# yifita/iso-points

Hardware: AMD Instinct MI355X
Metric: Mpoints/s full iso-point cycle (project+resample+splat), 1M pts (higher is better)
Workload: dtype f32-class (split-fp16 operands, 2^-22: hidden-layer products from two fp16 parts per f32 operand under exact power-of-two scales, 3 fp16-MFMA passes, f32 accumulate; everything else f32)

## Files before the change

include/isopoints.h:

```cpp
#ifndef ISOPOINTS_H_
#define ISOPOINTS_H_

#include <stdint.h>

#ifdef __cplusplus
extern "C" {
#endif

#define ISO_OK 0
#define ISO_ERR_INVALID (-1)
#define ISO_ERR_UNSUPPORTED (-2)
#define ISO_ERR_LAUNCH (-3)
#define ISO_ERR_WORKSPACE (-4)

const char* iso_version(void);
const char* iso_last_error(void);


int iso_project_sphere(const float* pts_in, float* pts_out, float* normals_out,
                       uint8_t* mask_out, int64_t n, float cx, float cy,
                       float cz, float radius, int max_iters, float tol,
                       void* stream);

typedef struct iso_follow {
// ... 297 lines not shown
int iso_bricks_box_take(void* workspace, int64_t n_max, float* box_out, void* stream);
int iso_bricks_build(const float* points, const float* normals, const int32_t* payload,
                     int64_t n_own, int64_t id_base, const float* import_rec0,
                     const float* import_rec1, const int32_t* import_count, int64_t import_max,
                     const float* bbox, int64_t n_total, float radius, int knn_k,
                     float cell_scale, void* workspace, int64_t workspace_bytes, void* stream);
int iso_bricks_params(const float* boxes, int n_boxes, int64_t n_total, int64_t n_own, int64_t id_base, float radius,
                      int knn_k, float cell_scale, void* workspace, int64_t n_max, void* stream);
int iso_halo_export(void* workspace, const float* points, const float* normals, const int32_t* payload,
                    int64_t n_own, const float* rank_boxes, int world, int rank, int halo_cells,
                    float* export_buf, int64_t capacity, void* stream);
int iso_halo_import(void* workspace, int64_t n_max, const float* gathered, const float* rank_boxes, int world,
                    int rank, int halo_cells, int64_t capacity, float* import_rec0, float* import_rec1,
                    int32_t* import_count, int64_t import_capacity, void* stream);
int iso_resample_fused(void* workspace, int64_t n_max, const float* points, int64_t n_own,
                       int k_plus_one, float* points_out, int64_t* idx_out, float* d2_out,
                       void* stream);
int iso_splat_view_mask(const float* points, const float* normals, const float* views, int n_views,
                        int64_t n, float znear, float zfar, int backface_culling,
                        int32_t* mask_out, int32_t* view_count_out, void* stream);
int iso_splat_h_fused(void* workspace, int64_t n_max, const float* points, const int32_t* mask,
                      int64_t n_own, const int32_t* view_total, int n_views, float* h_out,
                      void* stream);
int64_t iso_splat_front_workspace_bytes(int64_t n_points);
int iso_splat_front(const float* points, const float* normals, const float* features, int channels,
                    int features_from_normals, const int32_t* mask, const float* h, int64_t n_points,
                    const float* views, const float* projs, int n_views, int image_size, float sigma,
                    float cutoff, void* workspace, int64_t workspace_bytes, int64_t* first_idx_out,
                    int64_t* num_pts_out, int32_t* view_total_out, float* ndc_out, float* ellipse_out,
                    float* cutoff_out, float* radii_out, float* scaler_out, float* features_out,
                    int32_t* src_out, void* stream);
int iso_splat_view_mask_scan(const float* points, const float* normals, const float* views, int n_views,
                             int64_t n_points, float znear, float zfar, int backface_culling, int32_t* mask_out,
                             void* workspace, int64_t workspace_bytes, int64_t* first_idx_out, int64_t* num_pts_out,
                             int32_t* view_total_out, void* stream);
int iso_splat_front_rows(const float* points, const float* normals, const float* features, int channels,
                         int features_from_normals, const int32_t* mask, const float* h, int64_t n_points,
                         const float* views, const float* projs, int n_views, int image_size, float sigma,
                         float cutoff, const void* workspace, int64_t workspace_bytes, const int64_t* first_idx,
                         float* ndc_out, float* ellipse_out, float* cutoff_out, float* radii_out,
                         float* scaler_out, float* features_out, int32_t* src_out,
                         uint8_t* visible_zero_out ,
                         int64_t row_capacity ,
                         int32_t* overflow_out ,
                         void* stream);
int iso_splat_points_backward(const float* points, int64_t n_points, const float* views, const float* projs,
// ... 129 lines not shown
```

iso_points_amd/_lib.py:

```python
import ctypes
import os

import torch

_HERE = os.path.dirname(os.path.abspath(__file__))
LIB_PATH = os.path.join(_HERE, "libisopoints_hip.so")
if os.environ.get("ISO_DEV_LIB"):
    LIB_PATH = os.path.abspath(os.environ["ISO_DEV_LIB"])

_c = ctypes
_P = _c.c_void_p
_I = _c.c_int
_L = _c.c_int64
_F = _c.c_float

SIGNATURES = {
    "iso_version": (_c.c_char_p, []),
    "iso_last_error": (_c.c_char_p, []),
    "iso_project_sphere": (_I, [_P, _P, _P, _P, _L, _F, _F, _F, _F, _I, _F, _P]),
    "iso_project_sphere_follow": (_I, [_P, _P, _P, _P, _L, _F, _F, _F, _F, _I, _F, _P, _P]),
    "iso_siren_raw_floats": (_L, [_I, _I]),
    "iso_siren_packed_floats": (_L, [_I, _I]),
    "iso_siren_set_gemm_mode": (_I, [_I]),
    "iso_siren_get_gemm_mode": (_I, []),
# ... 66 lines not shown
                                      _L, _P, _P, _I, _I, _F, _P, _P, _P]),
    "iso_gather_neg_idx": (_I, [_P, _P, _L, _P, _P]),
    "iso_splat_composite": (_I, [_P, _P, _P, _P, _P, _L, _I, _I, _I, _F, _P, _P, _P]),
    "iso_splat_composite_backward": (_I, [_P, _P, _P, _P, _P, _L, _I, _I, _I, _F, _P, _P, _P, _P, _P]),
    "iso_splat_mark_visible": (_I, [_P, _L, _I, _P, _P]),
    "iso_splat_median_radius_workspace_bytes": (_L, [_I]),
    "iso_splat_median_radius": (_I, [_P, _P, _P, _P, _I, _L, _F, _P, _L, _P, _P]),
    "iso_splat_backward_workspace_bytes": (_L, [_I, _I, _I, _L]),
    "iso_splat_backward": (_I, [_P, _P, _P, _P, _P, _P, _I, _L, _P, _P, _P, _I, _I, _I, _I, _F, _L, _P, _L, _P, _P]),
    "iso_splat_zbuf_backward": (_I, [_P, _P, _L, _I, _P, _P]),
    "iso_bricks_workspace_bytes": (_L, [_L]),
    "iso_bricks_workspace_init": (_I, [_P, _L, _P]),
    "iso_bricks_workspace_check": (_I, [_P, _L, _P]),
    "iso_bricks_build_whole": (_I, [_P, _P, _P, _L, _F, _I, _F, _P, _L, _P]),
    "iso_bricks_build_pending": (_I, [_P, _P, _P, _L, _F, _I, _F, _P, _L, _P, _P]),
    "iso_bricks_box_take": (_I, [_P, _L, _P, _P]),
    "iso_bricks_build": (_I, [_P, _P, _P, _L, _L, _P, _P, _P, _L, _P, _L, _F, _I, _F, _P, _L, _P]),
    "iso_bricks_params": (_I, [_P, _I, _L, _L, _L, _F, _I, _F, _P, _L, _P]),
    "iso_halo_export": (_I, [_P, _P, _P, _P, _L, _P, _I, _I, _I, _P, _L, _P]),
    "iso_halo_import": (_I, [_P, _L, _P, _P, _I, _I, _I, _L, _P, _P, _P, _L, _P]),
    "iso_resample_fused": (_I, [_P, _L, _P, _L, _I, _P, _P, _P, _P]),
    "iso_splat_view_mask": (_I, [_P, _P, _P, _I, _L, _F, _F, _I, _P, _P, _P]),
    "iso_splat_h_fused": (_I, [_P, _L, _P, _P, _L, _P, _I, _P, _P]),
    "iso_splat_z_absmax": (_I, [_P, _L, _P, _P]),
    "iso_splat_z_scatter": (_I, [_P, _P, _L, _I, _L, _P, _P, _P]),
    "iso_splat_z_finish": (_I, [_P, _P, _L, _L, _P, _P]),
    "iso_splat_band_marks": (_I, [_P, _P, _I, _L, _L, _I, _P, _P, _P]),
    "iso_splat_band_z_scatter": (_I, [_P, _P, _I, _L, _L, _I, _P, _P, _P]),
    "iso_splat_repack": (_I, [_P, _L, _I, _I, _I, _P, _F, _L, _P, _P, _P, _P, _P, _P, _P, _P, _P, _P, _P]),
    "iso_splat_band_segment_floats": (_L, [_L]),
    "iso_splat_band_export_workspace_bytes": (_L, [_L, _I, _I]),
    "iso_splat_band_export": (_I, [_P, _P, _P, _P, _P, _P, _P, _I, _L, _P, _I, _I, _I, _I, _L, _P, _P, _P, _P, _P, _P, _P, _P,
                                   _P, _L, _P]),
    "iso_splat_band_import": (_I, [_P, _I, _I, _L, _L, _F, _P, _P, _P, _P, _P, _P, _P, _P, _P, _P, _P, _P, _P, _P, _P]),
    "iso_splat_band_remap": (_I, [_P, _P, _I, _L, _L, _L, _I, _P, _P]),
    "iso_splat_band_return": (_I, [_P, _P, _P, _P, _P, _I, _L, _P, _P]),
    "iso_splat_band_merge": (_I, [_P, _P, _I, _I, _L, _L, _P, _P, _P, _P]),
    "iso_splat_median_pass_words": (_L, [_I]),
    "iso_splat_median_pass": (_I, [_I, _P, _P, _P, _P, _I, _L, _P, _L, _P]),
    "iso_splat_median_final": (_I, [_P, _I, _F, _P, _P]),
    "iso_insert_fathers": (_I, [_P, _P, _I, _L, _P, _P, _P, _P, _P]),
    "iso_insert_children": (_I, [_P, _P, _I, _L, _I, _I, _P, _P, _P, _P, _P]),
    "iso_splat_points_backward": (_I, [_P, _L, _P, _P, _I, _P, _P, _P, _P, _P, _P, _P]),
    "iso_rasterize_coarse": (_I, [_P, _P, _P, _P, _I, _I, _I, _I, _P, _P, _P]),
    "iso_rasterize_fine": (_I, [_P, _P, _P, _P, _L, _P, _I, _I, _F, _I, _I, _I, _P, _P, _P, _P, _P]),
    "iso_splat_front_workspace_bytes": (_L, [_L]),
# ... 86 lines not shown
```

iso_points_amd/bricks.py:

```python
import torch

from . import _lib

RESAMPLE_CELL = 0.8
H_CELL_SCALE = 6.0


def points_bbox(points, out=None):
    pts = points.detach().float().contiguous().view(-1, 3)
    mm = out if out is not None else torch.empty((8,), dtype=torch.float32, device=pts.device)
    _lib.call("iso_points_bbox", _lib.ptr(pts), None, 1, pts.shape[0], _lib.ptr(mm), _lib.stream())
    return mm


class BrickGrid(object):

    def __init__(self, n_own, device, import_max=0):
        self.n_own, self.import_max = int(n_own), int(import_max)
        self.n_max = self.n_own + self.import_max
        lib = _lib.load()
        self.ws_bytes = lib.iso_bricks_workspace_bytes(self.n_max)
        self.ws = torch.empty((self.ws_bytes,), dtype=torch.uint8, device=device)
        assert self.ws.data_ptr() % 256 == 0
        _lib.call("iso_bricks_workspace_init", _lib.ptr(self.ws), self.n_max, _lib.stream())
# ... 36 lines not shown
                  p(self.ws), self.ws_bytes, _lib.stream())
        self.points = points
        self._imports = imports
        return self

    def counters_since_last(self):
        c = self.ws[256:384].cpu().view(torch.int32).tolist()
        tot = [(c[i] + c[16 + i]) & 0xffffffff for i in range(16)]
        out = [(tot[i] - self._seen[i]) & 0xffffffff for i in range(16)]
        self._seen = tot
        return out

    def check_initialised(self):
        _lib.call("iso_bricks_workspace_check", _lib.ptr(self.ws), self.n_max, _lib.stream())

    def header(self):
        self.check_initialised()
        raw = self.ws[:128].cpu()
        f = raw.view(torch.float32).tolist()
        i = raw.view(torch.int32).tolist()
        c = self.ws[256:320].cpu().view(torch.int32).tolist()
        return {"f": f[8], "r": f[9], "inv_sigma": f[12], "diag": f[13], "nb": i[16:19], "n_bricks": i[19],
                "n": i[23], "n_own": i[24], "id_base": i[25], "g_covers_r": i[26], "occupied": c[0],
                "tail": c[1], "overflow_bricks": c[2], "tail_h": c[3]}


class Follow(object):

    def __init__(self, grid, n, views=None, znear=1.0, zfar=100.0, backface_culling=True):
        dev = grid.ws.device
        self.grid, self.n = grid, int(n)
        self.done = False
        self.views = None
        self.mask = self.total = self.scanned = None
        self.znear, self.zfar, self.backface = float(znear), float(zfar), bool(backface_culling)
        if views is not None:
            nv = views.shape[0]
            self.views = views.detach().float().contiguous()
            self.mask = torch.empty((self.n,), dtype=torch.int32, device=dev)
            ws = torch.empty((_lib.load().iso_splat_front_workspace_bytes(self.n),), dtype=torch.uint8, device=dev)
            first = torch.empty((nv,), dtype=torch.int64, device=dev)
            num = torch.empty((nv,), dtype=torch.int64, device=dev)
            self.total = torch.empty((8,), dtype=torch.int32, device=dev)
            self.scanned = (ws, first, num, self.total)

    def struct(self):
        p = lambda t: (t.data_ptr() if t is not None else None)
# ... 64 lines not shown
```

iso_points_amd/csrc/bricks.hip:

```cpp
#include <type_traits>
#include "bricks.h"

#pragma clang fp contract(off)

constexpr int kScan1MaxWords = 2048;
BrickWs bricks_carve(void* ws, int64_t n_max) {
  BrickWs w;
  if (n_max < 1) n_max = 1;
  w.nb_cap = bricks_nb_cap(n_max);
  w.G = BK_CPB * (int64_t)w.nb_cap * w.nb_cap * w.nb_cap + 1;
  auto al = [](int64_t b) { return (b + 255) / 256 * 256; };
  char* p = (char*)ws;
  int64_t o = 0;
  w.hdr = (BrickHdr*)(p + o); o += al(sizeof(BrickHdr));
  w.counters = (int32_t*)(p + o); o += al(4 * kCounterInts);
  w.scan1 = (unsigned*)(p + o); o += al(4 * kScan1MaxWords);
  w.cnt = (int32_t*)(p + o); o += al(4 * w.G);
  w.off = (int32_t*)(p + o); o += al(4 * w.G);
  w.slot = (int32_t*)(p + o); o += al(4 * n_max);
  w.rec0 = (float4*)(p + o); o += al(16 * n_max);
  w.rec1 = (float4*)(p + o); o += al(16 * n_max);
  w.list = (int32_t*)(p + o); o += al(4 * (w.G < n_max ? w.G : n_max));
  w.tail = (int32_t*)(p + o); o += al(4 * 8 * n_max);
  w.scan_ws_bytes = iso_prefix_sum_workspace_bytes(w.G, 1) + 4 * (kScan1MaxWords + (w.G + 1023) / 1024);
// ... 666 lines not shown
  constexpr int NL = BrickStage<WITH_NRM, 2>::NL;
  int cell = (wx * NL + wy) * NL + wz;
  int i = S.cstart[cell], e = S.cstart[cell + NW];
  cell += NL;
  int ni = S.cstart[cell], ne = S.cstart[cell + NW];
  int run = 0, m = 1;
  while (run < NW * NW) {
    const bool v0 = i < e, v1 = i + 1 < e;
    const int i0 = v0 ? i : 0, i1 = v1 ? i + 1 : i0;
    const float4 c0 = S.rec0[i0];
    const float4 c1 = S.rec0[i1];
    body(c0, i0, c1, i1, v0, v1);
    i += 2;
    if (i >= e) {
      ++run;
      i = ni; e = ne;
      m = m == NW - 1 ? 0 : m + 1;
      cell += m == 0 ? NL * NL - (NW - 1) * NL : NL;
      if (run < NW * NW - 1) { ni = S.cstart[cell]; ne = S.cstart[cell + NW]; }
    }
  }
}

__device__ void brick_to_tail(const BrickHdr& h, const int32_t* __restrict__ off, const float4* __restrict__ rec0, int b,
                              int32_t* __restrict__ tail, int32_t* __restrict__ counters, int tail_slot, int per_query) {
  for (int i = off[BK_CPB * b] + threadIdx.x; i < off[BK_CPB * (b + 1)]; i += BK_THREADS) {
    const int gid = __float_as_int(rec0[i].w);
    if (gid >= h.id_base && gid < h.id_base + h.n_own) {
      const int at = atomicAdd(&counters[tail_slot], per_query);
      for (int v = 0; v < per_query; ++v) tail[at + v] = per_query > 1 ? (gid - h.id_base) * 8 + v : gid - h.id_base;
    }
  }
  if (threadIdx.x == 0) atomicAdd(&counters[2], 1);
}

struct Repulse {
  float px, py, pz, inv_sigma;
  float sw = 0.f, mx = 0.f, my = 0.f, mz = 0.f;
  __device__ __forceinline__ void add(float qx, float qy, float qz, float ux, float uy, float uz) {
    const float dx = px - qx, dy = py - qy, dz = pz - qz;
    const float d2 = (dx * dx + dy * dy) + dz * dz;
    const float w = expf(-d2 * inv_sigma);
    const float dn = (dx * ux + dy * uy) + dz * uz;
    const float tx = dx - dn * ux, ty = dy - dn * uy, tz = dz - dn * uz;
    sw += w;
    mx += w * tx; my += w * ty; mz += w * tz;
  }
  __device__ __forceinline__ void finish(float* __restrict__ o) const {
    const float dens = sw + 1.0f;
    const float den = iso_eps_denom(sw, 1.0e-17f);
    o[0] = px + dens * mx / den;
    o[1] = py + dens * my / den;
    o[2] = pz + dens * mz / den;
  }
};

__device__ __forceinline__ bool pair_lt(float d1, int i1, float d2, int i2) {
  return d1 < d2 || (d1 == d2 && i1 < i2);
}

constexpr int kXcdChunks = 8;
__device__ __forceinline__ int bk_xcd_span(int n_list) {
  return kXcdChunks * ((n_list + kXcdChunks - 1) / kXcdChunks);
}
__device__ __forceinline__ int bk_xcd_item(int lj, int n_list) {
  const int chunk = (n_list + kXcdChunks - 1) / kXcdChunks;
  return (lj % kXcdChunks) * chunk + lj / kXcdChunks;
}

template <int M>
__global__ __launch_bounds__(BK_THREADS, 4) void k_brick_resample(
    const BrickHdr* __restrict__ hp, const int32_t* __restrict__ off, const int32_t* __restrict__ list,
    const float4* __restrict__ rec0, const float4* __restrict__ rec1, int K, float* __restrict__ out,
    int64_t* __restrict__ idx_out, float* __restrict__ d2_out, int32_t* __restrict__ tail,
    int32_t* __restrict__ counters) {
  __shared__ BrickStage<true, 2> S;
  __shared__ int s_unc[BK_THREADS], s_nunc;
  const BrickHdr h = *hp;
  const int n_list = counters[0];
  for (int lj = blockIdx.x; lj < bk_xcd_span(n_list); lj += gridDim.x) {
    const int li = bk_xcd_item(lj, n_list);
    if (li >= n_list) continue;
    const int b = list[li];
    BrickGeo g;
    if (threadIdx.x == 0) s_nunc = 0;
    const int C = stage_brick<true, 1, 2>(S, h, off, rec0, rec1, b, g);
    if (C < 0) { brick_to_tail(h, off, rec0, b, tail, counters, 1, 1); continue; }
    const int nq = S.qpre[BrickStage<true, 2>::NQRUN];
    auto one_query = [&](int pos, auto wide_tag) -> bool {
      constexpr bool WIDE = decltype(wide_tag)::value;
      constexpr int ML = (WIDE && M == 10) ? 12 : M;
      const float4 q = S.rec0[pos];
      const int gid = __float_as_int(q.w);
      int wx, wy, wz;
      float mfrac = 0.f;
      {
        auto win = [&](float pc, float mn, int nf, int o) {
          const float t2 = ((pc - mn) * h.inv_f) * 2.0f;
          int sc = (int)floorf(t2);
          sc = sc < 0 ? 0 : (sc >= 2 * nf ? 2 * nf - 1 : sc);
          if (WIDE) return 2 * (sc >> 1) - 2 * o - 2;
          const float fr = t2 - (float)sc;
          const bool low = fr < 0.5f;
          mfrac = fmaxf(mfrac, low ? fr : 1.0f - fr);
          return sc - 2 * o - (low ? 2 : 1);
        };
        wx = win(q.x, h.mn[0], h.nf[0], g.ox);
        wy = win(q.y, h.mn[1], h.nf[1], g.oy);
        wz = win(q.z, h.mn[2], h.nf[2], g.oz);
      }
      float gq2 = h.g2;
      if (!WIDE) { const float gq = (2.0f - mfrac) * 0.5f; gq2 = (gq * gq) * h.g2; }
      unsigned key[ML];
#pragma unroll
      for (int j = 0; j < ML; ++j) key[j] = 0xffffffffu;
      auto visit = [&](const float4& c0, int i0, const float4& c1, int i1, bool v0, bool v1) {
        const float da = bk_d2(q.x, q.y, q.z, c0.x, c0.y, c0.z);
        const float db = bk_d2(q.x, q.y, q.z, c1.x, c1.y, c1.z);
        const unsigned ka = v0 ? ((__float_as_uint(da) & ~1023u) | (unsigned)i0) : 0xffffffffu;
        const unsigned kb = v1 ? ((__float_as_uint(db) & ~1023u) | (unsigned)i1) : 0xffffffffu;
#pragma unroll
        for (int j = ML - 1; j >= 1; --j) key[j] = bk_med3u(key[j - 1], ka, key[j]);
        key[0] = min(key[0], ka);
#pragma unroll
        for (int j = ML - 1; j >= 1; --j) key[j] = bk_med3u(key[j - 1], kb, key[j]);
        key[0] = min(key[0], kb);
      };
      if (WIDE) walk_window<6>(S, wx, wy, wz, visit);
      else walk_window_flat<4>(S, wx, wy, wz, visit);
      float d[ML];
      int id[ML], ps[ML];
#pragma unroll
      for (int j = 0; j < ML; ++j) {
        const bool valid = key[j] != 0xffffffffu;
        ps[j] = valid ? (int)(key[j] & 1023u) : pos;
        const float4 c = S.rec0[ps[j]];
        const float d2 = bk_d2(q.x, q.y, q.z, c.x, c.y, c.z);
        const bool ok = valid && d2 < h.r2;
        d[j] = ok ? d2 : FLT_MAX;
        id[j] = ok ? __float_as_int(c.w) : 0x7fffffff;
      }
      bool swapped;
      do {
        swapped = false;
#pragma unroll
        for (int j = 0; j + 1 < ML; ++j) {
          if (pair_lt(d[j + 1], id[j + 1], d[j], id[j])) {
            const float td = d[j]; d[j] = d[j + 1]; d[j + 1] = td;
            const int ti = id[j]; id[j] = id[j + 1]; id[j + 1] = ti;
            const int tp = ps[j]; ps[j] = ps[j + 1]; ps[j + 1] = tp;
            swapped = true;
// ... 20 lines not shown
          if (j < ML && j < K && d[j < ML ? j : 0] < FLT_MAX) u[k] = rec1[S.src[ps[j < ML ? j : 0]]];
        }
#pragma unroll
        for (int k = 0; k < 4; ++k) {
          const int j = j0 + k;
          if (j < ML && j < K && d[j < ML ? j : 0] < FLT_MAX) {
            const float4 c = S.rec0[ps[j < ML ? j : 0]];
            R.add(c.x, c.y, c.z, u[k].x, u[k].y, u[k].z);
          }
        }
      }
      R.finish(out + (int64_t)row * 3);
      if (idx_out) {
#pragma unroll
        for (int j = 1; j < ML; ++j)
          if (j < K) {
            idx_out[(int64_t)row * (K - 1) + j - 1] = d[j] < FLT_MAX ? (int64_t)id[j] : (int64_t)-1;
            if (d2_out) d2_out[(int64_t)row * (K - 1) + j - 1] = d[j] < FLT_MAX ? d[j] : -1.0f;
          }
      }
      return true;
    };
    auto to_tail = [&](int pos) { tail[atomicAdd(&counters[1], 1)] = __float_as_int(S.rec0[pos].w) - h.id_base; };
    for (int t = threadIdx.x; t < nq; t += BK_THREADS) {
      const int pos = query_slot(S, t);
      const int gid = __float_as_int(S.rec0[pos].w);
      if (gid < h.id_base || gid >= h.id_base + h.n_own) continue;
      if (!one_query(pos, std::false_type())) {
        const int at = atomicAdd(&s_nunc, 1);
        if (at < BK_THREADS) s_unc[at] = pos; else to_tail(pos);
      }
    }
    __syncthreads();
    const int n_unc = min(s_nunc, BK_THREADS);
    for (int u = threadIdx.x; u < n_unc; u += BK_THREADS) {
      const int pos = s_unc[u];
      if (!one_query(pos, std::true_type())) to_tail(pos);
    }
  }
}

struct WalkGeo { float qx, qy, qz, mnx, mny, mnz, B; };
constexpr int kWalkItems = 8;

template <class Fetch, class Body, class Bound, class Local>
__device__ __forceinline__ void bk_walk_shell(int rin, int rho, int qbx, int qby, int qbz, int nbx, int nby, int nbz,
                                              const int32_t* __restrict__ off, int lane, const WalkGeo& G,
                                              Fetch&& fetch, Body&& body, Bound&& bound, Local&& local,
                                              int part = 0, int nparts = 1) {
  const int x0 = max(qbx - rho, 0), x1 = min(qbx + rho, nbx - 1);
  const int y0 = max(qby - rho, 0), y1 = min(qby + rho, nby - 1);
  if (x0 > x1 || y0 > y1) return;
  const int ny = y1 - y0 + 1, ncols = (x1 - x0 + 1) * ny;
  for (int c0 = 0; c0 < ncols; c0 += 64) {
    int s0 = 0, e0 = 0, s1 = 0, e1 = 0;
    float dm0 = FLT_MAX, dm1 = FLT_MAX;
    const int col = c0 + lane;
    const float far2 = bound();
    auto gap = [&](float q, float mn, int b0, int b1) {
      const float lo = mn + (float)b0 * G.B, hi = mn + (float)(b1 + 1) * G.B;
// ... 215 lines not shown
  for (int v = 0; v < 8; ++v) {
    if (v < n_views) {
      int c = local[v];
#pragma unroll
      for (int o = 32; o > 0; o >>= 1) c += __shfl_xor(c, o);
      if ((threadIdx.x & 63) == 0 && c) atomicAdd(&s_cnt[v], c);
    }
  }
  __syncthreads();
  if (threadIdx.x < n_views && s_cnt[threadIdx.x]) atomicAdd(&view_count[threadIdx.x], s_cnt[threadIdx.x]);
}

__device__ __forceinline__ float h_from_list(const float* d , bool small_cloud) {
  float m = -FLT_MAX;
#pragma unroll
  for (int k = 1; k < 7; ++k) {
    const float v = small_cloud ? 1e-3f : (d[k] < FLT_MAX ? d[k] : -1.0f);
    m = fmaxf(m, v);
  }
  return fminf(fmaxf(0.5f * m, 5e-5f), 0.01f);
}

constexpr int kHWgs = 6;
template <int NV>
__global__ __launch_bounds__(BK_THREADS, NV <= 4 ? kHWgs : 4) void k_brick_h(
    const BrickHdr* __restrict__ hp, const int32_t* __restrict__ off, const int32_t* __restrict__ list,
    const float4* __restrict__ rec0, const float4* __restrict__ rec1, const int32_t* __restrict__ view_total,
    int n_views, float* __restrict__ h_out , int32_t* __restrict__ tail,
    int32_t* __restrict__ counters) {
  __shared__ BrickStage<false, 1, BK_CAP> S;
  const BrickHdr h = *hp;
  const int n_list = counters[0];
  bool small_cloud[NV];
#pragma unroll
  for (int v = 0; v < NV; ++v) small_cloud[v] = v < n_views && view_total[v] < 7;
  const float kT = 2.0f * 5e-5f;
  const float t2 = fminf(kT, h.r2 > 0.f ? __uint_as_float(__float_as_uint(h.r2) - 1u) : 0.f);
  for (int lj = blockIdx.x; lj < bk_xcd_span(n_list); lj += gridDim.x) {
    const int li = bk_xcd_item(lj, n_list);
    if (li >= n_list) continue;
    const int b = list[li];
    BrickGeo g;
    constexpr int VS = NV <= 4 ? 8 : 1;
    const int C = stage_brick<false, VS, 1, BK_CAP>(S, h, off, rec0, rec1, b, g);
    if (C < 0) { brick_to_tail(h, off, rec0, b, tail, counters, 3, 8); continue; }
    const int nq = S.qpre[16];
    for (int t0 = 0; t0 < nq; t0 += BK_THREADS) {
      const int t = t0 + threadIdx.x;
      float4 q = make_float4(0.f, 0.f, 0.f, 0.f);
      int qmask = 0, lx = 1, ly = 1, lz = 1, row = 0, sx = 1, sy = 1;
      if (t < nq) {
        const int pos = query_slot(S, t);
        q = S.rec0[pos];
        qmask = __float_as_int(q.w);
        if (qmask < 0) qmask = 0;
        row = S.gid[pos] - h.id_base;
        const int fx = bk_fine(q.x, h.mn[0], h.inv_f, h.nf[0]), fy = bk_fine(q.y, h.mn[1], h.inv_f, h.nf[1]);
        lx = fx - g.ox;
        ly = fy - g.oy;
        lz = bk_fine(q.z, h.mn[2], h.inv_f, h.nf[2]) - g.oz;
        sx = ((q.x - h.mn[0]) * h.inv_f - (float)fx) >= 0.5f ? 1 : -1;
        sy = ((q.y - h.mn[1]) * h.inv_f - (float)fy) >= 0.5f ? 1 : -1;
      }
      int cnt[NV];
#pragma unroll
      for (int v = 0; v < NV; ++v) cnt[v] = 0;
      if (VS == 8 && C <= 255) {
        unsigned acc = 0;
        const unsigned need = ((unsigned)qmask & 0x01010101u) << 7;
        if (qmask)
          walk_candidates_near_first(S, lx, ly, lz, sx, sy, [&](const float4& c0, const float4& c1, bool v0, bool v1) {
            const float da = bk_d2(q.x, q.y, q.z, c0.x, c0.y, c0.z);
            const float db = bk_d2(q.x, q.y, q.z, c1.x, c1.y, c1.z);
            const unsigned ma = (v0 && da <= t2) ? (__float_as_uint(c0.w) & 0x01010101u) : 0u;
            const unsigned mb = (v1 && db <= t2) ? (__float_as_uint(c1.w) & 0x01010101u) : 0u;
            acc += ma + mb;
          }, [&]() {
            const unsigned ge7 = (((acc & 0x7f7f7f7fu) + 0x79797979u) | acc) & 0x80808080u;
            return (ge7 & need) == need;
          });
#pragma unroll
        for (int v = 0; v < NV; ++v) cnt[v] = (int)((acc >> (8 * (v & 3))) & 0xffu);
      } else if (qmask)
        walk_candidates_near_first(S, lx, ly, lz, sx, sy, [&](const float4& c0, const float4& c1, bool v0, bool v1) {
          const float da = bk_d2(q.x, q.y, q.z, c0.x, c0.y, c0.z);
          const float db = bk_d2(q.x, q.y, q.z, c1.x, c1.y, c1.z);
          const int ma = (v0 && da <= t2) ? __float_as_int(c0.w) : 0;
          const int mb = (v1 && db <= t2) ? __float_as_int(c1.w) : 0;
#pragma unroll
          for (int v = 0; v < NV; ++v) cnt[v] += ((ma >> (VS * v)) & 1) + ((mb >> (VS * v)) & 1);
        }, [&]() {
          bool all = true;
#pragma unroll
          for (int v = 0; v < NV; ++v) all = all && (!((qmask >> (VS * v)) & 1) || cnt[v] >= 7);
          return all;
        });
      bool open_ = false;
#pragma unroll
      for (int v = 0; v < NV; ++v) open_ = open_ || (((qmask >> (VS * v)) & 1) && !small_cloud[v] && cnt[v] < 7);
      float d[NV][7];
#pragma unroll
      for (int v = 0; v < NV; ++v)
#pragma unroll
        for (int j = 0; j < 7; ++j) d[v][j] = FLT_MAX;
      if (open_)
        walk_candidates(S, lx, ly, lz, [&](const float4& c0, const float4& c1, bool v0, bool v1) {
          float da = bk_d2(q.x, q.y, q.z, c0.x, c0.y, c0.z);
          float db = bk_d2(q.x, q.y, q.z, c1.x, c1.y, c1.z);
          da = (v0 && da < h.r2) ? da : FLT_MAX;
          db = (v1 && db < h.r2) ? db : FLT_MAX;
          const int ma = __float_as_int(c0.w), mb = __float_as_int(c1.w);
#pragma unroll
          for (int v = 0; v < NV; ++v) {
            const float ka = (ma >> (VS * v)) & 1 ? da : FLT_MAX;
            const float kb = (mb >> (VS * v)) & 1 ? db : FLT_MAX;
#pragma unroll
            for (int j = 6; j >= 1; --j) d[v][j] = __builtin_amdgcn_fmed3f(d[v][j - 1], ka, d[v][j]);
            d[v][0] = fminf(d[v][0], ka);
#pragma unroll
            for (int j = 6; j >= 1; --j) d[v][j] = __builtin_amdgcn_fmed3f(d[v][j - 1], kb, d[v][j]);
            d[v][0] = fminf(d[v][0], kb);
          }
        });
      if (qmask) {
#pragma unroll
        for (int v = 0; v < NV; ++v) {
          if (v < n_views && ((qmask >> (VS * v)) & 1)) {
            float hv;
            bool cert = true;
            if (small_cloud[v]) hv = fminf(fmaxf(0.5f * 1e-3f, 5e-5f), 0.01f);
            else if (cnt[v] >= 7) hv = 5e-5f;
            else {
              cert = h.g_covers_r || (d[v][6] < FLT_MAX && d[v][6] <= h.g2);
              hv = h_from_list(d[v], false);
            }
            if (cert) h_out[(int64_t)v * h.n_own + row] = hv;
            else tail[atomicAdd(&counters[3], 1)] = row * 8 + v;
          }
        }
      }
    }
  }
}

template <int KMAX>
struct TopF {
  float d[KMAX];
// ... 417 lines not shown
  ISO_REQUIRE(workspace && gathered && rank_boxes && import_rec0 && import_rec1 && import_count && world >= 1 &&
                  rank >= 0 && rank < world && capacity >= 0 && import_capacity >= 0 && halo_cells >= 1,
              ISO_ERR_INVALID, "iso_halo_import: bad arguments");
  const BrickWs w = bricks_carve(workspace, n_max);
  hipStream_t s = (hipStream_t)stream;
  iso_zero_words(import_count, 1, s);
  if (capacity > 0 && world > 1)
    hipLaunchKernelGGL(k_halo_import, dim3(iso_stream_grid(capacity, 256) > 64 ? 64 : iso_stream_grid(capacity, 256), world),
                       dim3(256), 0, s, (const float4*)gathered, world, rank, (int)capacity, halo_cells, w.hdr, rank_boxes,
                       (float4*)import_rec0, (float4*)import_rec1, import_count, (int)import_capacity, w.counters);
  ISO_CHECK_LAUNCH("iso_halo_import");
  return ISO_OK;
}

static int brick_grid(int64_t n_own, int cap) {
  int64_t g = n_own / 48;
  if (g < 1024) g = 1024;
  if (g > cap) g = cap;
  return (int)g;
}
static int h_grid(int64_t n_own) { return brick_grid(n_own, 10240); }
static int resample_grid(int64_t n_own) { return brick_grid(n_own, 8192); }

extern "C" int iso_resample_fused(void* workspace, int64_t n_max, const float* points, int64_t n_own,
                                  int k_plus_one, float* points_out, int64_t* idx_out, float* d2_out,
                                  void* stream) {
  ISO_REQUIRE(workspace && n_own >= 0 && n_max >= n_own, ISO_ERR_INVALID, "iso_resample_fused: bad arguments");
  ISO_REQUIRE(k_plus_one >= 2 && k_plus_one <= 13, ISO_ERR_UNSUPPORTED,
              "iso_resample_fused: K + 1 must be in [2,13], got %d", k_plus_one);
  if (n_own == 0) return ISO_OK;
  ISO_REQUIRE(points && points_out && points != points_out, ISO_ERR_INVALID, "iso_resample_fused: null / aliased pointer");
  const BrickWs w = bricks_carve(workspace, n_max);
  hipStream_t s = (hipStream_t)stream;
  const int K = k_plus_one;
#define ISO_RS(MM)                                                                                           \
  hipLaunchKernelGGL(k_brick_resample<MM>, dim3(resample_grid(n_own)), dim3(BK_THREADS), 0, s, w.hdr, w.off, w.list, \
                     w.rec0, w.rec1, K, points_out, idx_out, d2_out, w.tail, w.counters)
  if (K <= 5) ISO_RS(8);
  else if (K == 9) ISO_RS(10);
  else if (K <= 9) ISO_RS(12);
  else ISO_RS(16);
#undef ISO_RS
  int tb = (int)(n_own < 4096 ? n_own : 4096);
  hipLaunchKernelGGL(k_brick_resample_tail<16>, dim3(tb), dim3(64), 0, s, w.hdr, w.off, w.rec0, w.rec1, points, K,
                     points_out, idx_out, d2_out, w.tail, w.counters);
  ISO_CHECK_LAUNCH("iso_resample_fused");
  return ISO_OK;
}

extern "C" int iso_splat_view_mask(const float* points, const float* normals, const float* views, int n_views,
                                   int64_t n, float znear, float zfar, int backface_culling, int32_t* mask_out,
                                   int32_t* view_count_out, void* stream) {
  ISO_REQUIRE(n >= 0 && n_views >= 1 && n_views <= 8, ISO_ERR_UNSUPPORTED, "iso_splat_view_mask: 1..8 views per call");
  ISO_REQUIRE(views && mask_out && view_count_out && (points || n == 0) && (normals || !backface_culling),
              ISO_ERR_INVALID, "iso_splat_view_mask: null pointer");
  hipStream_t s = (hipStream_t)stream;
  iso_zero_words(view_count_out, 8, s);
  if (n > 0)
    hipLaunchKernelGGL(k_view_mask, dim3(iso_stream_grid(n, 256 * 4)), dim3(256), 0, s, points, normals, views, n_views,
                       n, znear, zfar, backface_culling, mask_out, view_count_out);
  ISO_CHECK_LAUNCH("iso_splat_view_mask");
  return ISO_OK;
}

extern "C" int iso_splat_h_fused(void* workspace, int64_t n_max, const float* points, const int32_t* mask,
                                 int64_t n_own, const int32_t* view_total, int n_views, float* h_out,
                                 void* stream) {
  ISO_REQUIRE(workspace && n_own >= 0 && n_max >= n_own, ISO_ERR_INVALID, "iso_splat_h_fused: bad arguments");
  ISO_REQUIRE(n_views >= 1 && n_views <= 8, ISO_ERR_UNSUPPORTED, "iso_splat_h_fused: 1..8 views per call");
  if (n_own == 0) return ISO_OK;
  ISO_REQUIRE(points && mask && view_total && h_out, ISO_ERR_INVALID, "iso_splat_h_fused: null pointer");
  const BrickWs w = bricks_carve(workspace, n_max);
  hipStream_t s = (hipStream_t)stream;
#define ISO_H(NV)                                                                                            \
  hipLaunchKernelGGL(k_brick_h<NV>, dim3(h_grid(n_own)), dim3(BK_THREADS), 0, s, w.hdr, w.off, w.list, w.rec0, \
                     w.rec1, view_total, n_views, h_out, w.tail, w.counters)
  if (n_views <= 1) ISO_H(1);
  else if (n_views <= 2) ISO_H(2);
  else if (n_views <= 4) ISO_H(4);
  else ISO_H(8);
#undef ISO_H
  if (n_own < kTailWideBelow)
    hipLaunchKernelGGL((k_brick_h_tail<2 * kHTailWaves>), dim3(4096), dim3(64 * 2 * kHTailWaves), 0, s, w.hdr, w.off, w.rec0, w.rec1, points, mask, view_total,
                     n_views, h_out, w.tail, w.counters);
  else
    hipLaunchKernelGGL((k_brick_h_tail<kHTailWaves>), dim3(4096), dim3(64 * kHTailWaves), 0, s, w.hdr, w.off, w.rec0, w.rec1, points, mask, view_total,
                     n_views, h_out, w.tail, w.counters);
  ISO_CHECK_LAUNCH("iso_splat_h_fused");
  return ISO_OK;
}
```

Measured before the change: 73.54.

## Split each brick query across paired lanes with DPP merging in resample and h

When a brick holds at most half a block's worth of queries, each query is now handled by two adjacent lanes. Each lane walks alternating candidates, and the partial top-k keys or neighbour counts are merged through a DPP lane swap. This applies to the resample kNN kernel and to the splat-h kernel, and is meant to fill lanes that otherwise sit idle on sparsely populated bricks. It adds more template instantiations and extra merge work, and brings register-pressure risk. A runtime mask enables the path per kernel (default: resample only) and can optionally count which form each brick used.

Result: no change. 73.43 (-0.2%).

```diff
diff --git a/include/isopoints.h b/include/isopoints.h
--- a/include/isopoints.h
+++ b/include/isopoints.h
@@ -343,6 +343,7 @@
 int iso_splat_h_fused(void* workspace, int64_t n_max, const float* points, const int32_t* mask,
                       int64_t n_own, const int32_t* view_total, int n_views, float* h_out,
                       void* stream);
+int iso_bricks_set_pair_lanes(int mask);
 int64_t iso_splat_front_workspace_bytes(int64_t n_points);
 int iso_splat_front(const float* points, const float* normals, const float* features, int channels,
                     int features_from_normals, const int32_t* mask, const float* h, int64_t n_points,
diff --git a/iso_points_amd/_lib.py b/iso_points_amd/_lib.py
--- a/iso_points_amd/_lib.py
+++ b/iso_points_amd/_lib.py
@@ -112,6 +112,7 @@
     "iso_resample_fused": (_I, [_P, _L, _P, _L, _I, _P, _P, _P, _P]),
     "iso_splat_view_mask": (_I, [_P, _P, _P, _I, _L, _F, _F, _I, _P, _P, _P]),
     "iso_splat_h_fused": (_I, [_P, _L, _P, _P, _L, _P, _I, _P, _P]),
+    "iso_bricks_set_pair_lanes": (_I, [_I]),
     "iso_splat_z_absmax": (_I, [_P, _L, _P, _P]),
     "iso_splat_z_scatter": (_I, [_P, _P, _L, _I, _L, _P, _P, _P]),
     "iso_splat_z_finish": (_I, [_P, _P, _L, _L, _P, _P]),
diff --git a/iso_points_amd/bricks.py b/iso_points_amd/bricks.py
--- a/iso_points_amd/bricks.py
+++ b/iso_points_amd/bricks.py
@@ -82,7 +82,20 @@
         c = self.ws[256:320].cpu().view(torch.int32).tolist()
         return {"f": f[8], "r": f[9], "inv_sigma": f[12], "diag": f[13], "nb": i[16:19], "n_bricks": i[19],
                 "n": i[23], "n_own": i[24], "id_base": i[25], "g_covers_r": i[26], "occupied": c[0],
-                "tail": c[1], "overflow_bricks": c[2], "tail_h": c[3]}
+                "tail": c[1], "overflow_bricks": c[2], "tail_h": c[3], "two_lane_bricks": c[7], "one_lane_bricks": c[8]}
+
+    def tail_list(self, bandwidth=False):
+        al = lambda b: (b + 255) // 256 * 256
+        n = max(self.n_max, 1)
+        cap = 8
+        while cap * cap * 64 < n and cap < 160:
+            cap += 1
+        G = 8 * cap ** 3 + 1
+        at = al(128) + al(4 * 576) + al(4 * 2048) + 2 * al(4 * G) + al(4 * n) + 2 * al(16 * n) + al(4 * min(G, n))
+        scan = _lib.load().iso_prefix_sum_workspace_bytes(G, 1) + 4 * (2048 + (G + 1023) // 1024)
+        assert at + al(32 * n) + al(scan) == self.ws_bytes, "tail_list no longer mirrors bricks_carve"
+        count = self.header()["tail_h" if bandwidth else "tail"]
+        return self.ws[at:at + 4 * count].cpu().view(torch.int32)
 
 
 class Follow(object):
diff --git a/iso_points_amd/csrc/bricks.hip b/iso_points_amd/csrc/bricks.hip
--- a/iso_points_amd/csrc/bricks.hip
+++ b/iso_points_amd/csrc/bricks.hip
@@ -712,6 +712,64 @@
   }
 }
 
+__device__ __forceinline__ unsigned bk_pair_u(unsigned v) {
+  return (unsigned)__builtin_amdgcn_update_dpp(0, (int)v, 0xB1 , 0xF, 0xF, false);
+}
+__device__ __forceinline__ float bk_pair_f(float v) { return __uint_as_float(bk_pair_u(__float_as_uint(v))); }
+
+template <int R, int W, bool TIE, class St, class CellAt, class Body, class Done>
+__device__ __forceinline__ void walk_ranges_pair(const St& S, int part, CellAt&& cell_at, Body&& body, Done&& done) {
+  int c = cell_at(0);
+  int i = S.cstart[c], e = S.cstart[c + W];
+  c = cell_at(1);
+  int ni = S.cstart[c], ne = S.cstart[c + W];
+  int run = 0;
+  auto step = [&]() {
+    i += 2;
+    if (i >= e) {
+      ++run;
+      i = ni; e = ne;
+      if (run < R - 1) { const int cn = cell_at(run + 1); ni = S.cstart[cn]; ne = S.cstart[cn + W]; }
+    }
+  };
+  while (run < R) {
+    const int ia = i, ea = e;
+    step();
+    const bool live = part ? run < R : true;
+    const int it = part ? i : ia, et = part ? e : ea;
+    const bool v0 = live && it < et, v1 = live && it + 1 < et;
+    const int i0 = v0 ? it : 0, i1 = v1 ? it + 1 : i0;
+    float4 c0 = S.rec0[i0];
+    float4 c1 = S.rec0[i1];
+    if (TIE) asm volatile("" : "+v"(c0.x), "+v"(c0.y), "+v"(c0.z), "+v"(c0.w), "+v"(c1.x), "+v"(c1.y), "+v"(c1.z), "+v"(c1.w));
+    body(c0, i0, c1, i1, v0, v1);
+    step();
+    if (done()) run = R;
+  }
+}
+
+template <int NW, bool WITH_NRM, class Body>
+__device__ __forceinline__ void walk_window_pair(const BrickStage<WITH_NRM, 2>& S, int wx, int wy, int wz, int part, Body&& body) {
+  constexpr int NL = BrickStage<WITH_NRM, 2>::NL;
+  auto cell0 = [&](int c) { return ((wx + c / NW) * NL + (wy + c % NW)) * NL + wz; };
+  int a = S.cstart[cell0(0)], e = S.cstart[cell0(0) + NW];
+  int o = 2 * part;
+  for (int c = 0; c < NW * NW; ++c) {
+    int na = 0, ne = 0;
+    if (c < NW * NW - 1) { na = S.cstart[cell0(c + 1)]; ne = S.cstart[cell0(c + 1) + NW]; }
+    int i = a + o;
+    for (; i < e; i += 4) {
+      const bool two = i + 1 < e;
+      const int i1 = two ? i + 1 : i;
+      const float4 c0 = S.rec0[i];
+      const float4 c1 = S.rec0[i1];
+      body(c0, i, c1, i1, true, two);
+    }
+    o = (i - e) & 2;
+    a = na; e = ne;
+  }
+}
+
 __device__ void brick_to_tail(const BrickHdr& h, const int32_t* __restrict__ off, const float4* __restrict__ rec0, int b,
                               int32_t* __restrict__ tail, int32_t* __restrict__ counters, int tail_slot, int per_query) {
   for (int i = off[BK_CPB * b] + threadIdx.x; i < off[BK_CPB * (b + 1)]; i += BK_THREADS) {
@@ -758,12 +816,12 @@
   return (lj % kXcdChunks) * chunk + lj / kXcdChunks;
 }
 
-template <int M>
+template <int M, bool TWO>
 __global__ __launch_bounds__(BK_THREADS, 4) void k_brick_resample(
     const BrickHdr* __restrict__ hp, const int32_t* __restrict__ off, const int32_t* __restrict__ list,
     const float4* __restrict__ rec0, const float4* __restrict__ rec1, int K, float* __restrict__ out,
     int64_t* __restrict__ idx_out, float* __restrict__ d2_out, int32_t* __restrict__ tail,
-    int32_t* __restrict__ counters) {
+    int32_t* __restrict__ counters, int count_forms) {
   __shared__ BrickStage<true, 2> S;
   __shared__ int s_unc[BK_THREADS], s_nunc;
   const BrickHdr h = *hp;
@@ -777,8 +835,11 @@
     const int C = stage_brick<true, 1, 2>(S, h, off, rec0, rec1, b, g);
     if (C < 0) { brick_to_tail(h, off, rec0, b, tail, counters, 1, 1); continue; }
     const int nq = S.qpre[BrickStage<true, 2>::NQRUN];
-    auto one_query = [&](int pos, auto wide_tag) -> bool {
+    const bool two = TWO && nq <= BK_THREADS / 2;
+    if (count_forms && threadIdx.x == 0) atomicAdd(&counters[two ? 7 : 8], 1);
+    auto one_query = [&](int pos, auto wide_tag, auto pair_tag, int part) -> bool {
       constexpr bool WIDE = decltype(wide_tag)::value;
+      constexpr bool PAIR = decltype(pair_tag)::value;
       constexpr int ML = (WIDE && M == 10) ? 12 : M;
       const float4 q = S.rec0[pos];
       const int gid = __float_as_int(q.w);
@@ -816,7 +877,24 @@
         for (int j = ML - 1; j >= 1; --j) key[j] = bk_med3u(key[j - 1], kb, key[j]);
         key[0] = min(key[0], kb);
       };
-      if (WIDE) walk_window<6>(S, wx, wy, wz, visit);
+      if (PAIR) {
+        if (WIDE) walk_window_pair<6>(S, wx, wy, wz, part, visit);
+        else {
+          constexpr int NL = BrickStage<true, 2>::NL;
+          const int cell = (wx * NL + wy) * NL + wz;
+          walk_ranges_pair<16, 4, false>(S, part, [&](int k) { return cell + (k >> 2) * (NL * NL) + (k & 3) * NL; }, visit,
+                                  []() { return false; });
+        }
+#pragma unroll
+        for (int k = 0; k < ML; ++k) {
+          unsigned kp = bk_pair_u(key[k]);
+          if (part) kp = 0xffffffffu;
+#pragma unroll
+          for (int j = ML - 1; j >= 1; --j) key[j] = bk_med3u(key[j - 1], kp, key[j]);
+          key[0] = min(key[0], kp);
+        }
+        if (part) return true;
+      } else if (WIDE) walk_window<6>(S, wx, wy, wz, visit);
       else walk_window_flat<4>(S, wx, wy, wz, visit);
       float d[ML];
       int id[ML], ps[ML];
@@ -883,20 +961,41 @@
       return true;
     };
     auto to_tail = [&](int pos) { tail[atomicAdd(&counters[1], 1)] = __float_as_int(S.rec0[pos].w) - h.id_base; };
-    for (int t = threadIdx.x; t < nq; t += BK_THREADS) {
-      const int pos = query_slot(S, t);
-      const int gid = __float_as_int(S.rec0[pos].w);
-      if (gid < h.id_base || gid >= h.id_base + h.n_own) continue;
-      if (!one_query(pos, std::false_type())) {
-        const int at = atomicAdd(&s_nunc, 1);
-        if (at < BK_THREADS) s_unc[at] = pos; else to_tail(pos);
+    auto queue_wide = [&](int pos) {
+      const int at = atomicAdd(&s_nunc, 1);
+      if (at < BK_THREADS) s_unc[at] = pos; else to_tail(pos);
+    };
+    int pt = threadIdx.x;
+    if (M < 16) asm volatile("" : "+v"(pt));
+    if (two) {
+      const int t = pt >> 1;
+      if (t < nq) {
+        const int pos = query_slot(S, t);
+        const int gid = __float_as_int(S.rec0[pos].w);
+        if (gid >= h.id_base && gid < h.id_base + h.n_own)
+          if (!one_query(pos, std::false_type(), std::true_type(), pt & 1)) queue_wide(pos);
+      }
+    } else {
+      for (int t = threadIdx.x; t < nq; t += BK_THREADS) {
+        const int pos = query_slot(S, t);
+        const int gid = __float_as_int(S.rec0[pos].w);
+        if (gid < h.id_base || gid >= h.id_base + h.n_own) continue;
+        if (!one_query(pos, std::false_type(), std::false_type(), 0)) queue_wide(pos);
       }
     }
     __syncthreads();
     const int n_unc = min(s_nunc, BK_THREADS);
-    for (int u = threadIdx.x; u < n_unc; u += BK_THREADS) {
-      const int pos = s_unc[u];
-      if (!one_query(pos, std::true_type())) to_tail(pos);
+    if (TWO && n_unc <= BK_THREADS / 2) {
+      const int u = pt >> 1;
+      if (u < n_unc) {
+        const int pos = s_unc[u];
+        if (!one_query(pos, std::true_type(), std::true_type(), pt & 1)) to_tail(pos);
+      }
+    } else {
+      for (int u = threadIdx.x; u < n_unc; u += BK_THREADS) {
+        const int pos = s_unc[u];
+        if (!one_query(pos, std::true_type(), std::false_type(), 0)) to_tail(pos);
+      }
     }
   }
 }
@@ -1158,12 +1257,12 @@
 }
 
 constexpr int kHWgs = 6;
-template <int NV>
+template <int NV, bool TWO>
 __global__ __launch_bounds__(BK_THREADS, NV <= 4 ? kHWgs : 4) void k_brick_h(
     const BrickHdr* __restrict__ hp, const int32_t* __restrict__ off, const int32_t* __restrict__ list,
     const float4* __restrict__ rec0, const float4* __restrict__ rec1, const int32_t* __restrict__ view_total,
     int n_views, float* __restrict__ h_out , int32_t* __restrict__ tail,
-    int32_t* __restrict__ counters) {
+    int32_t* __restrict__ counters, int count_forms) {
   __shared__ BrickStage<false, 1, BK_CAP> S;
   const BrickHdr h = *hp;
   const int n_list = counters[0];
@@ -1181,8 +1280,12 @@
     const int C = stage_brick<false, VS, 1, BK_CAP>(S, h, off, rec0, rec1, b, g);
     if (C < 0) { brick_to_tail(h, off, rec0, b, tail, counters, 3, 8); continue; }
     const int nq = S.qpre[16];
+    const bool two = TWO && nq <= BK_THREADS / 2;
+    if (count_forms && threadIdx.x == 0) atomicAdd(&counters[two ? 7 : 8], 1);
+    const int part = two ? (int)(threadIdx.x & 1) : 0;
+    constexpr int NL = BrickStage<false, 1, BK_CAP>::NL;
     for (int t0 = 0; t0 < nq; t0 += BK_THREADS) {
-      const int t = t0 + threadIdx.x;
+      const int t = two ? (int)(threadIdx.x >> 1) : t0 + (int)threadIdx.x;
       float4 q = make_float4(0.f, 0.f, 0.f, 0.f);
       int qmask = 0, lx = 1, ly = 1, lz = 1, row = 0, sx = 1, sy = 1;
       if (t < nq) {
@@ -1201,7 +1304,53 @@
       int cnt[NV];
 #pragma unroll
       for (int v = 0; v < NV; ++v) cnt[v] = 0;
-      if (VS == 8 && C <= 255) {
+      auto near_cell = [&](int k) {
+        constexpr unsigned KA = 1u | 2u << 2 | 1u << 4 | 2u << 6 | 0u << 8 | 1u << 10 | 0u << 12 | 2u << 14 | 0u << 16;
+        constexpr unsigned KB = 1u | 1u << 2 | 2u << 4 | 2u << 6 | 1u << 8 | 0u << 10 | 2u << 12 | 0u << 14 | 0u << 16;
+        const int a = (int)((KA >> (2 * k)) & 3u) - 1, b = (int)((KB >> (2 * k)) & 3u) - 1;
+        return (lx * NL + ly) * NL + (lz - 1) + a * (sx * NL * NL) + b * (sy * NL);
+      };
+      if (TWO && two) {
+        if (VS == 8 && C <= 255) {
+          unsigned acc = 0;
+          const unsigned need = ((unsigned)qmask & 0x01010101u) << 7;
+          if (qmask)
+            walk_ranges_pair<9, 3, true>(S, part, near_cell, [&](const float4& c0, int, const float4& c1, int, bool v0, bool v1) {
+              const float da = bk_d2(q.x, q.y, q.z, c0.x, c0.y, c0.z);
+              const float db = bk_d2(q.x, q.y, q.z, c1.x, c1.y, c1.z);
+              const unsigned ma = (v0 && da <= t2) ? (__float_as_uint(c0.w) & 0x01010101u) : 0u;
+              const unsigned mb = (v1 && db <= t2) ? (__float_as_uint(c1.w) & 0x01010101u) : 0u;
+              acc += ma + mb;
+            }, [&]() {
+              const unsigned sum = acc + bk_pair_u(acc);
+              const unsigned ge7 = (((sum & 0x7f7f7f7fu) + 0x79797979u) | sum) & 0x80808080u;
+              return (ge7 & need) == need;
+            });
+          acc += bk_pair_u(acc);
+#pragma unroll
+          for (int v = 0; v < NV; ++v) cnt[v] = (int)((acc >> (8 * (v & 3))) & 0xffu);
+        } else {
+          if (qmask)
+            walk_ranges_pair<9, 3, true>(S, part, near_cell, [&](const float4& c0, int, const float4& c1, int, bool v0, bool v1) {
+              const float da = bk_d2(q.x, q.y, q.z, c0.x, c0.y, c0.z);
+              const float db = bk_d2(q.x, q.y, q.z, c1.x, c1.y, c1.z);
+              const int ma = (v0 && da <= t2) ? __float_as_int(c0.w) : 0;
+              const int mb = (v1 && db <= t2) ? __float_as_int(c1.w) : 0;
+#pragma unroll
+              for (int v = 0; v < NV; ++v) cnt[v] += ((ma >> (VS * v)) & 1) + ((mb >> (VS * v)) & 1);
+            }, [&]() {
+              bool all = true;
+#pragma unroll
+              for (int v = 0; v < NV; ++v) {
+                const int sum = cnt[v] + (int)bk_pair_u((unsigned)cnt[v]);
+                all = all & (!((qmask >> (VS * v)) & 1) | (sum >= 7));
+              }
+              return all;
+            });
+#pragma unroll
+          for (int v = 0; v < NV; ++v) cnt[v] += (int)bk_pair_u((unsigned)cnt[v]);
+        }
+      } else if (VS == 8 && C <= 255) {
         unsigned acc = 0;
         const unsigned need = ((unsigned)qmask & 0x01010101u) << 7;
         if (qmask)
@@ -1239,26 +1388,41 @@
       for (int v = 0; v < NV; ++v)
 #pragma unroll
         for (int j = 0; j < 7; ++j) d[v][j] = FLT_MAX;
-      if (open_)
-        walk_candidates(S, lx, ly, lz, [&](const float4& c0, const float4& c1, bool v0, bool v1) {
-          float da = bk_d2(q.x, q.y, q.z, c0.x, c0.y, c0.z);
-          float db = bk_d2(q.x, q.y, q.z, c1.x, c1.y, c1.z);
-          da = (v0 && da < h.r2) ? da : FLT_MAX;
-          db = (v1 && db < h.r2) ? db : FLT_MAX;
-          const int ma = __float_as_int(c0.w), mb = __float_as_int(c1.w);
+      auto push = [&](int v, float k) {
+#pragma unroll
+        for (int j = 6; j >= 1; --j) d[v][j] = __builtin_amdgcn_fmed3f(d[v][j - 1], k, d[v][j]);
+        d[v][0] = fminf(d[v][0], k);
+      };
+      auto visit2 = [&](const float4& c0, const float4& c1, bool v0, bool v1) {
+        float da = bk_d2(q.x, q.y, q.z, c0.x, c0.y, c0.z);
+        float db = bk_d2(q.x, q.y, q.z, c1.x, c1.y, c1.z);
+        da = (v0 && da < h.r2) ? da : FLT_MAX;
+        db = (v1 && db < h.r2) ? db : FLT_MAX;
+        const int ma = __float_as_int(c0.w), mb = __float_as_int(c1.w);
+#pragma unroll
+        for (int v = 0; v < NV; ++v) {
+          push(v, (ma >> (VS * v)) & 1 ? da : FLT_MAX);
+          push(v, (mb >> (VS * v)) & 1 ? db : FLT_MAX);
+        }
+      };
+      if (TWO && two) {
+        if (open_) {
+          const int cell = ((lx - 1) * NL + (ly - 1)) * NL + (lz - 1);
+          walk_ranges_pair<9, 3, true>(S, part, [&](int k) { const int kx = (k * 11) >> 5; return cell + kx * (NL * NL) + (k - 3 * kx) * NL; },
+                                 [&](const float4& c0, int, const float4& c1, int, bool v0, bool v1) { visit2(c0, c1, v0, v1); },
+                                 []() { return false; });
 #pragma unroll
           for (int v = 0; v < NV; ++v) {
-            const float ka = (ma >> (VS * v)) & 1 ? da : FLT_MAX;
-            const float kb = (mb >> (VS * v)) & 1 ? db : FLT_MAX;
-#pragma unroll
-            for (int j = 6; j >= 1; --j) d[v][j] = __builtin_amdgcn_fmed3f(d[v][j - 1], ka, d[v][j]);
-            d[v][0] = fminf(d[v][0], ka);
-#pragma unroll
-            for (int j = 6; j >= 1; --j) d[v][j] = __builtin_amdgcn_fmed3f(d[v][j - 1], kb, d[v][j]);
-            d[v][0] = fminf(d[v][0], kb);
+            float dp[7];
+#pragma unroll
+            for (int j = 0; j < 7; ++j) dp[j] = bk_pair_f(d[v][j]);
+#pragma unroll
+            for (int j = 0; j < 7; ++j) push(v, dp[j]);
           }
-        });
-      if (qmask) {
+        }
+      } else if (open_)
+        walk_candidates(S, lx, ly, lz, visit2);
+      if (qmask && !part) {
 #pragma unroll
         for (int v = 0; v < NV; ++v) {
           if (v < n_views && ((qmask >> (VS * v)) & 1)) {
@@ -1722,6 +1886,17 @@
 static int h_grid(int64_t n_own) { return brick_grid(n_own, 10240); }
 static int resample_grid(int64_t n_own) { return brick_grid(n_own, 8192); }
 
+constexpr int kPairLanesDefault = 1;
+static int g_pair_lanes = -1;
+static int pair_mask() { return g_pair_lanes < 0 ? kPairLanesDefault : g_pair_lanes; }
+static bool pair_lanes(int bit) { return (pair_mask() & bit) != 0; }
+static int count_forms() { return (pair_mask() & 4) ? 1 : 0; }
+extern "C" int iso_bricks_set_pair_lanes(int mask) {
+  ISO_REQUIRE(mask >= -1 && mask <= 7, ISO_ERR_INVALID, "iso_bricks_set_pair_lanes: -1 (default) or a mask in 0..7");
+  g_pair_lanes = mask;
+  return ISO_OK;
+}
+
 extern "C" int iso_resample_fused(void* workspace, int64_t n_max, const float* points, int64_t n_own,
                                   int k_plus_one, float* points_out, int64_t* idx_out, float* d2_out,
                                   void* stream) {
@@ -1733,14 +1908,17 @@
   const BrickWs w = bricks_carve(workspace, n_max);
   hipStream_t s = (hipStream_t)stream;
   const int K = k_plus_one;
-#define ISO_RS(MM)                                                                                           \
-  hipLaunchKernelGGL(k_brick_resample<MM>, dim3(resample_grid(n_own)), dim3(BK_THREADS), 0, s, w.hdr, w.off, w.list, \
-                     w.rec0, w.rec1, K, points_out, idx_out, d2_out, w.tail, w.counters)
+  const bool two = pair_lanes(1);
+#define ISO_RS1(MM, TWO)                                                                                     \
+  hipLaunchKernelGGL((k_brick_resample<MM, TWO>), dim3(resample_grid(n_own)), dim3(BK_THREADS), 0, s, w.hdr, w.off, w.list, \
+                     w.rec0, w.rec1, K, points_out, idx_out, d2_out, w.tail, w.counters, count_forms())
+#define ISO_RS(MM) do { if (two) ISO_RS1(MM, true); else ISO_RS1(MM, false); } while (0)
   if (K <= 5) ISO_RS(8);
   else if (K == 9) ISO_RS(10);
   else if (K <= 9) ISO_RS(12);
   else ISO_RS(16);
 #undef ISO_RS
+#undef ISO_RS1
   int tb = (int)(n_own < 4096 ? n_own : 4096);
   hipLaunchKernelGGL(k_brick_resample_tail<16>, dim3(tb), dim3(64), 0, s, w.hdr, w.off, w.rec0, w.rec1, points, K,
                      points_out, idx_out, d2_out, w.tail, w.counters);
@@ -1772,14 +1950,17 @@
   ISO_REQUIRE(points && mask && view_total && h_out, ISO_ERR_INVALID, "iso_splat_h_fused: null pointer");
   const BrickWs w = bricks_carve(workspace, n_max);
   hipStream_t s = (hipStream_t)stream;
-#define ISO_H(NV)                                                                                            \
-  hipLaunchKernelGGL(k_brick_h<NV>, dim3(h_grid(n_own)), dim3(BK_THREADS), 0, s, w.hdr, w.off, w.list, w.rec0, \
-                     w.rec1, view_total, n_views, h_out, w.tail, w.counters)
+  const bool two = pair_lanes(2);
+#define ISO_H1(NV, TWO)                                                                                      \
+  hipLaunchKernelGGL((k_brick_h<NV, TWO>), dim3(h_grid(n_own)), dim3(BK_THREADS), 0, s, w.hdr, w.off, w.list, w.rec0, \
+                     w.rec1, view_total, n_views, h_out, w.tail, w.counters, count_forms())
+#define ISO_H(NV) do { if (two) ISO_H1(NV, true); else ISO_H1(NV, false); } while (0)
   if (n_views <= 1) ISO_H(1);
   else if (n_views <= 2) ISO_H(2);
   else if (n_views <= 4) ISO_H(4);
   else ISO_H(8);
 #undef ISO_H
+#undef ISO_H1
   if (n_own < kTailWideBelow)
     hipLaunchKernelGGL((k_brick_h_tail<2 * kHTailWaves>), dim3(4096), dim3(64 * 2 * kHTailWaves), 0, s, w.hdr, w.off, w.rec0, w.rec1, points, mask, view_total,
                      n_views, h_out, w.tail, w.counters);
```
